# KerkDovan/univer-ocr

Measured on AMD Instinct MI355X. Metric: document-images/sec (fwd+bwd) on 256x512 synthetic pages, higher is better.
Workload: dtype f32; 1 GPU; BASELINE configs[2]: my_model train step (fwd+loss+bwd+L2+SGD) of Monochrome+Paragraph+Line on (32,256,512,1) pages and Char on (32,32,64,1) line strips per GPU; batch_per_gpu=32, global_batch=32, optimizer=sgd, parallelism=dp1, h2d_inclusive=False, input_grads=True, hip_graphs=True, pipelined_lanes=True, hw_queues=4

## Files before the change

include/univer_hip.h:

```cpp
#ifndef UNIVER_HIP_H
#define UNIVER_HIP_H

#include <stddef.h>
#include <stdint.h>

#ifdef __cplusplus
extern "C" {
#endif

#define UOCR_ABI_VERSION 4

typedef struct uocr_ctx uocr_ctx;

enum { UOCR_F32 = 0, UOCR_F64 = 1, UOCR_F16 = 2 };
#define UOCR_F16_SCALED(k) (UOCR_F16 | ((k) << 8))
#define UOCR_DTYPE_BASE(dtype) ((dtype) & 0xff)
#define UOCR_DTYPE_GRAD_SCALE_LOG2(dtype) (((dtype) >> 8) & 0xff)
enum { UOCR_ACT_NONE = 0, UOCR_ACT_RELU = 1, UOCR_ACT_LEAKY = 2, UOCR_ACT_SIGMOID = 3 };
enum { UOCR_LOSS_DICE = 0, UOCR_LOSS_JACCARD = 1 };
enum {
    UOCR_OK = 0,
    UOCR_ERR_ARG = -1,
    UOCR_ERR_DTYPE = -2,
    UOCR_ERR_HIP = -3,
    UOCR_ERR_WORKSPACE = -4,
    UOCR_ERR_UNSUPPORTED = -5,
    UOCR_ERR_RCCL = -6
};

int uocr_abi_version(void);
int uocr_ctx_create(int device, size_t workspace_bytes, uocr_ctx** out);
int uocr_ctx_create_cu_mask(int device, size_t workspace_bytes, const uint32_t* cu_mask, int mask_words, uocr_ctx** out);
int uocr_ctx_destroy(uocr_ctx* ctx);
int uocr_ctx_set_stream(uocr_ctx* ctx, void* hip_stream);
void* uocr_ctx_get_stream(uocr_ctx* ctx);
int uocr_ctx_set_option(uocr_ctx* ctx, const char* key, int value);
int uocr_ctx_last_split(uocr_ctx* ctx, int* blocks, long long* items);
int uocr_ctx_last_gemm(uocr_ctx* ctx, int* bm, int* gm, int* gn, int* nsplit);
int uocr_ctx_last_gemm_group(uocr_ctx* ctx, int* problems, int* split_problems);
int uocr_ctx_last_pair(uocr_ctx* ctx, int* kernel, int* g, int* mode, int* pf, int* nw, int* blocks_x, int* bands,
                       int* band_h);
enum {
    UOCR_CONV_NONE = 0,
    UOCR_CONV_GENERIC = 1,
    UOCR_CONV_MFMA = 2,
    UOCR_CONV_H16 = 3,
    UOCR_CONV_H16_WGRAD = 4,
    UOCR_CONV_H16_WGRAD_S2 = 5,
    UOCR_CONV_T32 = 6,
    UOCR_CONV_T32_WGRAD = 7,
    UOCR_CONV_H3 = 8,
    UOCR_CONV_TILED = 9,
    UOCR_CONV_C16_EXPAND = 10,
    UOCR_CONV_C16_REDUCE = 11,
    UOCR_CONV_C16_WGRAD = 12,
    UOCR_CONV_DGRAD_S2 = 13,
    UOCR_CONV_DGRAD_C64S2 = 14,
    UOCR_CONV_WGRAD_T542 = 15,
    UOCR_CONV_WGRAD_S2_TILED = 16,
    UOCR_CONV_TABLE_FAST = 17,
    UOCR_CONV_TABLE_PX = 18
};
int uocr_ctx_last_conv(uocr_ctx* ctx, int* entry, int* kernel);
int uocr_ctx_reserve_workspace(uocr_ctx* ctx, size_t bytes);
const char* uocr_last_error(uocr_ctx* ctx);
int uocr_malloc(uocr_ctx* ctx, size_t bytes, void** out);
int uocr_free(uocr_ctx* ctx, void* ptr);
int uocr_memset_zero(uocr_ctx* ctx, void* ptr, size_t bytes);
int uocr_h2d(uocr_ctx* ctx, void* dst, const void* src_host, size_t bytes);
int uocr_d2h_sync(uocr_ctx* ctx, void* dst_host, const void* src, size_t bytes);
int uocr_d2d(uocr_ctx* ctx, void* dst, const void* src, size_t bytes);
int uocr_stream_sync(uocr_ctx* ctx);
// ... 140 lines not shown
```

univer-ocr_amd/csrc/ctx.hip:

```cpp
#include <cstdlib>

#include "finish_group.h"
#include "gemm.h"
#include "uocr_common.h"

extern "C" {

int uocr_abi_version(void) { return UOCR_ABI_VERSION; }

int uocr_ctx_create(int device, size_t workspace_bytes, uocr_ctx** out) {
    if (!out || device < 0) return UOCR_ERR_ARG;
    *out = nullptr;
    int count = 0;
    if (hipGetDeviceCount(&count) != hipSuccess || device >= count) return UOCR_ERR_HIP;
    if (hipSetDevice(device) != hipSuccess) return UOCR_ERR_HIP;
    uocr_ctx* ctx = new uocr_ctx();
    ctx->device = device;
    ctx->err[0] = 0;
    ctx->workspace = nullptr;
    ctx->workspace_bytes = 0;
    ctx->sync = nullptr;
    ctx->gemm_defer = nullptr;
    ctx->snap_src = nullptr;
    ctx->snap_count = 0;
    ctx->snap_ring = nullptr;
    ctx->snap_ring_len = 0;
    ctx->snap_counter = nullptr;
    ctx->finish_defer = nullptr;
    ctx->owns_stream = true;
    ctx->opt_mfma = 1;
    ctx->opt_fast = 1;
    ctx->opt_tiled = 1;
    ctx->opt_split = 1024;
    ctx->opt_split_min = 3;
    ctx->opt_bm = 0;
    ctx->opt_h16 = 1;
    ctx->opt_t32 = 2;
    ctx->opt_xcd = 1;
    ctx->opt_pair_band = 0;
    ctx->opt_pair_g = 4;
    ctx->opt_group_blocks = 0;
    ctx->opt_wgrad_bands = 0;
    ctx->opt_max_blocks = 0;
    ctx->split_blocks = 0;
    ctx->split_items = 0;
    ctx->gemm_bm = ctx->gemm_gm = ctx->gemm_gn = ctx->gemm_nsplit = 0;
    ctx->gemm_group_count = ctx->gemm_group_split = 0;
    uocr_note_pair(ctx, 0, 0, 0, 0, 0, 0, 0, 0);
    uocr_note_conv(ctx, 0, UOCR_CONV_NONE);
    ctx->opt_h3 = 0;
#ifdef UOCR_EXPERIMENTS
    if (const char* e = getenv("UOCR_H3")) ctx->opt_h3 = atoi(e);
#endif
    ctx->opt_pair_pf = -1;
    if (const char* e = getenv("UOCR_PAIR_PF")) ctx->opt_pair_pf = atoi(e);
    if (const char* e = getenv("UOCR_WGRAD_BANDS")) ctx->opt_wgrad_bands = atoi(e);
    if (hipStreamCreateWithFlags(&ctx->stream, hipStreamNonBlocking) != hipSuccess) {
        delete ctx;
        return UOCR_ERR_HIP;
    }
    hipDeviceProp_t prop;
    ctx->cu_count = 256;
    if (hipGetDeviceProperties(&prop, device) == hipSuccess) ctx->cu_count = prop.multiProcessorCount;
    if (workspace_bytes) {
        if (hipMalloc(&ctx->workspace, workspace_bytes) != hipSuccess) {
            hipStreamDestroy(ctx->stream);
            delete ctx;
            return UOCR_ERR_HIP;
        }
        ctx->workspace_bytes = workspace_bytes;
    }
    if (hipMalloc((void**)&ctx->sync, UOCR_SYNC_WORDS * sizeof(unsigned)) != hipSuccess ||
        hipMemsetAsync(ctx->sync, 0, UOCR_SYNC_WORDS * sizeof(unsigned), ctx->stream) != hipSuccess ||
        hipStreamSynchronize(ctx->stream) != hipSuccess) {
        if (ctx->sync) hipFree(ctx->sync);
        if (ctx->workspace) hipFree(ctx->workspace);
        hipStreamDestroy(ctx->stream);
        delete ctx;
        return UOCR_ERR_HIP;
    }
// ... 22 lines not shown

int uocr_ctx_destroy(uocr_ctx* ctx) {
    UOCR_CHECK_CTX(ctx);
    hipSetDevice(ctx->device);
    hipStreamSynchronize(ctx->stream);
    if (ctx->workspace) hipFree(ctx->workspace);
    if (ctx->sync) hipFree(ctx->sync);
    uocr_gemm_defer_free(ctx);
    uocr_finish_defer_free(ctx);
    if (ctx->owns_stream) hipStreamDestroy(ctx->stream);
    delete ctx;
    return UOCR_OK;
}

int uocr_ctx_set_stream(uocr_ctx* ctx, void* hip_stream) {
    UOCR_CHECK_CTX(ctx);
    if (ctx->owns_stream) {
        UOCR_HIP(ctx, hipStreamSynchronize(ctx->stream));
        UOCR_HIP(ctx, hipStreamDestroy(ctx->stream));
        ctx->owns_stream = false;
    }
    ctx->stream = (hipStream_t)hip_stream;
    return UOCR_OK;
}

int uocr_ctx_set_option(uocr_ctx* ctx, const char* key, int value) {
    UOCR_CHECK_CTX(ctx);
    UOCR_REQUIRE(ctx, key != nullptr);
    if (!strcmp(key, "mfma")) ctx->opt_mfma = value;
    else if (!strcmp(key, "fast_paths")) ctx->opt_fast = value;
    else if (!strcmp(key, "tiled")) ctx->opt_tiled = value;
    else if (!strcmp(key, "split_blocks")) ctx->opt_split = value;
    else if (!strcmp(key, "split_min")) ctx->opt_split_min = value;
    else if (!strcmp(key, "gemm_bm")) ctx->opt_bm = value;
    else if (!strcmp(key, "xcd_remap")) ctx->opt_xcd = value;
    else if (!strcmp(key, "h16")) ctx->opt_h16 = value;
    else if (!strcmp(key, "t32")) {
        if (value & ~UOCR_T32_BUILT)
            UOCR_FAIL(ctx, UOCR_ERR_UNSUPPORTED, "option t32 = %d asks for kernels this library was built without "
                      "(UOCR_BUILD_EXPERIMENTS=1 ./build.sh)", value);
        ctx->opt_t32 = value;
    }
    else if (!strcmp(key, "pair_band")) ctx->opt_pair_band = value;
    else if (!strcmp(key, "pair_g")) ctx->opt_pair_g = value;
    else if (!strcmp(key, "group_blocks")) ctx->opt_group_blocks = value;
    else if (!strcmp(key, "wgrad_bands") && value >= 0) ctx->opt_wgrad_bands = value;
    else if (!strcmp(key, "max_blocks") && value >= 0) ctx->opt_max_blocks = value;
    else if (!strcmp(key, "h3")) {
#ifndef UOCR_EXPERIMENTS
        if (value) UOCR_FAIL(ctx, UOCR_ERR_UNSUPPORTED, "option h3: this library was built without conv_h3 "
                             "(UOCR_BUILD_EXPERIMENTS=1 ./build.sh)");
#endif
        ctx->opt_h3 = value;
    }
    else if (!strcmp(key, "pair_pf")) ctx->opt_pair_pf = value;
    else UOCR_FAIL(ctx, UOCR_ERR_ARG, "unknown option '%s'", key);
    return UOCR_OK;
}

int uocr_ctx_last_split(uocr_ctx* ctx, int* blocks, long long* items) {
    UOCR_CHECK_CTX(ctx);
    UOCR_REQUIRE(ctx, blocks && items);
    *blocks = ctx->split_blocks;
    *items = ctx->split_items;
    return UOCR_OK;
}

int uocr_ctx_last_gemm(uocr_ctx* ctx, int* bm, int* gm, int* gn, int* nsplit) {
    UOCR_CHECK_CTX(ctx);
    UOCR_REQUIRE(ctx, bm && gm && gn && nsplit);
    *bm = ctx->gemm_bm;
    *gm = ctx->gemm_gm;
    *gn = ctx->gemm_gn;
    *nsplit = ctx->gemm_nsplit;
    return UOCR_OK;
}

int uocr_ctx_last_gemm_group(uocr_ctx* ctx, int* problems, int* split_problems) {
    UOCR_CHECK_CTX(ctx);
    UOCR_REQUIRE(ctx, problems && split_problems);
    *problems = ctx->gemm_group_count;
    *split_problems = ctx->gemm_group_split;
    return UOCR_OK;
}

int uocr_ctx_last_pair(uocr_ctx* ctx, int* kernel, int* g, int* mode, int* pf, int* nw, int* blocks_x, int* bands,
                       int* band_h) {
    UOCR_CHECK_CTX(ctx);
    UOCR_REQUIRE(ctx, kernel && g && mode && pf && nw && blocks_x && bands && band_h);
    *kernel = ctx->pair_kernel;
    *g = ctx->pair_g;
    *mode = ctx->pair_mode;
    *pf = ctx->pair_pf;
    *nw = ctx->pair_nw;
    *blocks_x = ctx->pair_blocks_x;
    *bands = ctx->pair_bands;
    *band_h = ctx->pair_band_h;
    return UOCR_OK;
}

int uocr_ctx_last_conv(uocr_ctx* ctx, int* entry, int* kernel) {
    UOCR_CHECK_CTX(ctx);
    UOCR_REQUIRE(ctx, entry && kernel);
    *entry = ctx->conv_entry;
    *kernel = ctx->conv_kernel;
    return UOCR_OK;
}

void* uocr_ctx_get_stream(uocr_ctx* ctx) { return ctx ? (void*)ctx->stream : nullptr; }

int uocr_ctx_reserve_workspace(uocr_ctx* ctx, size_t bytes) {
    UOCR_CHECK_CTX(ctx);
    if (bytes <= ctx->workspace_bytes) return UOCR_OK;
    UOCR_HIP(ctx, hipSetDevice(ctx->device));
    UOCR_HIP(ctx, hipStreamSynchronize(ctx->stream));
    if (ctx->workspace) UOCR_HIP(ctx, hipFree(ctx->workspace));
    ctx->workspace = nullptr;
    ctx->workspace_bytes = 0;
// ... 146 lines not shown
```

univer-ocr_amd/csrc/gemm_mfma.hip:

```cpp
#include <array>
#include <type_traits>

#include "conv_dims.h"
#include "gemm.h"

namespace {

using f32x16 = __attribute__((ext_vector_type(16))) float;

constexpr int BN = 64;
constexpr int BD = 32;
constexpr int LDA = BD + 1;

struct alignas(16) F4 {
    float v[4];
};

__device__ __forceinline__ F4 f4_zero() { return F4{{0.f, 0.f, 0.f, 0.f}}; }
__device__ __forceinline__ F4 f4_fill(float x) { return F4{{x, x, x, x}}; }

enum : int { LD_KEEP = 0, LD_ZERO = 1, LD_E0 = 2, LD_PAD = 3 };

__device__ __forceinline__ F4 ld_resolve(F4 v, int code, float pad) {
    const float first = code == LD_PAD ? pad : (code == LD_E0 ? 1.f : 0.f);
    const float rest = code == LD_PAD ? pad : 0.f;
    F4 r;
    r.v[0] = code == LD_KEEP ? v.v[0] : first;
#pragma unroll
    for (int q = 1; q < 4; ++q) r.v[q] = code == LD_KEEP ? v.v[q] : rest;
    return r;
}

struct FastDiv {
    unsigned mul, shift;
    int d;
    FastDiv() = default;
    explicit FastDiv(int divisor) : mul(0), shift(0), d(divisor) {
        if (divisor > 1) {
            int lg = 0;
            while ((1ll << lg) < divisor) ++lg;
            const int p = 31 + lg;
// ... 306 lines not shown
            if (c.oy == d.oh) {
                c.oy = 0;
                c.b += 1;
                c.base += (d.h - d.oh * d.sh) * d.w * d.cin;
            }
        }
    }
    __device__ __forceinline__ F4 load_at(const Row& r, const Cursor& c, int& code) const {
        const int iy = c.oy * d.sh - d.ph + r.ky, ix = c.ox * d.sw - d.pw + r.kx;
        const bool inside = (unsigned)iy < (unsigned)d.h && (unsigned)ix < (unsigned)d.w;
        code = (c.b >= d.n || r.kind == 2) ? LD_ZERO : (r.kind == 1 ? LD_E0 : (inside ? LD_KEEP : LD_PAD));
        const int off = c.base + ((r.ky - d.ph) * d.w + (r.kx - d.pw)) * d.cin + r.ic0;
        return *reinterpret_cast<const F4*>(x + (code == LD_KEEP ? off : 0));
    }
};

template <int BM>
constexpr int gemm_a_floats() { return 2 * BM * LDA; }
template <typename BLoader>
constexpr int gemm_b_floats() { return 2 * (BLoader::DEPTH_CONTIG ? BN * LDA : BD * BN); }

__device__ __forceinline__ void gemm_block_coords(int lin, int gx, int gy, int gz, int xcd_remap, int& bx, int& by, int& bz) {
    if (xcd_remap) {
        const int total = gx * gy * gz;
        const int c = lin & 7, q = total >> 3, r = total & 7;
        lin = c * q + min(c, r) + (lin >> 3);
    }
    bx = lin % gx;
    const int rest = lin / gx;
    by = rest % gy;
    bz = rest / gy;
}

template <int BM, typename ALoader, typename BLoader>
__device__ __forceinline__ void gemm_tile(const ALoader& A, const BLoader& B, const Epilogue& ep, int M, int N, int ntiles,
                                          int tiles_per_split, float* slabs, int bx, int by, int bz, float* As,
                                          float* Bs) {
    constexpr int WM = BM / 32;
    constexpr int WN = 4 / WM;
    constexpr int NB = (BN / WN) / 32;
    constexpr int A_PASSES = BM / 32;
    constexpr int AM_GROUPS = BM / 4;
    constexpr int AM_ROWS = 256 / AM_GROUPS;
    constexpr int AM_PASSES = BD / AM_ROWS;
    constexpr int A_REGS = ALoader::DEPTH_CONTIG ? A_PASSES : AM_PASSES;
    constexpr int ASZ = BM * LDA;
    constexpr int BSZ = BLoader::DEPTH_CONTIG ? BN * LDA : BD * BN;

    const int tid = threadIdx.x, lane = tid & 63, wave = tid >> 6;
    const int m0 = bx * BM, n0 = by * BN;
    const int t_begin = bz * tiles_per_split;
    const int t_end = min(ntiles, t_begin + tiles_per_split);

    typename ALoader::Row rows[ALoader::DEPTH_CONTIG ? A_PASSES : 1];
    int a_kq = 0, a_r = 0, a_iq = 0, a_pr = 0;
    if constexpr (ALoader::DEPTH_CONTIG) {
        a_kq = tid & 7;
        a_r = tid >> 3;
#pragma unroll
        for (int s = 0; s < A_PASSES; ++s) rows[s] = A.prep(m0 + a_r + 32 * s);
    } else {
        a_iq = tid % AM_GROUPS;
        a_pr = tid / AM_GROUPS;
        rows[0] = A.prep(m0 + a_iq * 4);
    }
    const int b_nq = tid & 15, b_kr = tid >> 4;
    const int b_kq = tid & 7, b_r = tid >> 3;

    F4 areg[A_REGS], breg[2];
    int acode[A_REGS], bcode[2];
// ... 121 lines not shown
        if (band_live) {
            int ia = buf * ASZ + (ALoader::DEPTH_CONTIG ? fi * LDA + fk : fk * BM + fi);
            int ib = buf * BSZ + (BLoader::DEPTH_CONTIG ? fj * LDA + fk : fk * BN + fj);
            asm volatile("" : "+v"(ia), "+v"(ib));
            auto frag_a = [&](int k) { return As[ia + (ALoader::DEPTH_CONTIG ? k : k * BM)]; };
            auto frag_b = [&](int k, int nb) {
                return Bs[ib + (BLoader::DEPTH_CONTIG ? nb * 32 * LDA + k : k * BN + nb * 32)];
            };
            float a = frag_a(0), b[NB];
#pragma unroll
            for (int nb = 0; nb < NB; ++nb) b[nb] = frag_b(0, nb);
#pragma unroll
            for (int k = 0; k < BD; k += 2) {
                float an = 0.f, bn[NB];
                if (k + 2 < BD) {
                    an = frag_a(k + 2);
#pragma unroll
                    for (int nb = 0; nb < NB; ++nb) bn[nb] = frag_b(k + 2, nb);
                }
#pragma unroll
                for (int nb = 0; nb < NB; ++nb) acc[nb] = __builtin_amdgcn_mfma_f32_32x32x2f32(a, b[nb], acc[nb], 0, 0, 0);
                if (k + 2 < BD) {
                    a = an;
#pragma unroll
                    for (int nb = 0; nb < NB; ++nb) b[nb] = bn[nb];
                }
            }
        }
        if (more) store_tile(buf ^ 1);
        __syncthreads();
        t = tn;
    }

#pragma unroll
    for (int nb = 0; nb < NB; ++nb) {
        const int j = n0 + fj + nb * 32;
#pragma unroll
        for (int r = 0; r < 16; ++r) {
            const int i = m0 + wm * 32 + (r & 3) + 8 * (r >> 2) + 4 * (lane >> 5);
            if (i < M && j < N) {
                if (slabs) slabs[((long)bz * M + i) * N + j] = acc[nb][r];
                else epilogue_store(ep, i, j, acc[nb][r]);
            }
        }
    }
}

template <int BM, typename ALoader, typename BLoader>
__global__ __launch_bounds__(256) void mfma_gemm_kernel(ALoader A, BLoader B, Epilogue ep, int M, int N,
                                                        int ntiles, int tiles_per_split, float* slabs,
                                                        int xcd_remap) {
    __shared__ __attribute__((aligned(16))) float As[gemm_a_floats<BM>()];
    __shared__ __attribute__((aligned(16))) float Bs[gemm_b_floats<BLoader>()];
    int bx, by, bz;
    gemm_block_coords(blockIdx.x + gridDim.x * (blockIdx.y + gridDim.y * blockIdx.z), gridDim.x, gridDim.y, gridDim.z,
                      xcd_remap, bx, by, bz);
    gemm_tile<BM, ALoader, BLoader>(A, B, ep, M, N, ntiles, tiles_per_split, slabs, bx, by, bz, As, Bs);
}

__global__ __launch_bounds__(256) void slab_reduce_kernel(const float* __restrict__ slabs, int nsplit, int M, int N,
                                                          Epilogue ep) {
    const long total = (long)M * N;
    for (long idx = (long)blockIdx.x * blockDim.x + threadIdx.x; idx < total; idx += (long)gridDim.x * blockDim.x) {
        float v = 0.f;
        int z = 0;
        for (; z + 8 <= nsplit; z += 8) {
            float t[8];
#pragma unroll
            for (int k = 0; k < 8; ++k) t[k] = slabs[(long)(z + k) * total + idx];
#pragma unroll
            for (int k = 0; k < 8; ++k) v += t[k];
        }
        for (; z < nsplit; ++z) v += slabs[(long)z * total + idx];
        epilogue_store(ep, (int)(idx / N), (int)(idx % N), v);
    }
}

__global__ __launch_bounds__(256) void transpose_kernel(const float* __restrict__ in, float* __restrict__ out,
                                                        int rows, int cols) {
    const long total = (long)rows * cols;
    for (long idx = (long)blockIdx.x * blockDim.x + threadIdx.x; idx < total; idx += (long)gridDim.x * blockDim.x) {
        const int c = (int)(idx / rows), r = (int)(idx % rows);
        out[idx] = in[(long)r * cols + c];
    }
}

inline bool aligned16(const void* p) { return (reinterpret_cast<uintptr_t>(p) & 15u) == 0; }

inline float* ws_slabs(uocr_ctx* ctx) { return (float*)ctx->workspace; }
inline float* ws_aux(uocr_ctx* ctx) { return (float*)((char*)ctx->workspace + ctx->workspace_bytes / 2); }
inline size_t ws_half(uocr_ctx* ctx) { return ctx->workspace_bytes / 2; }

template <typename ALoader, typename BLoader>
int launch_mfma(uocr_ctx* ctx, const ALoader& A, const BLoader& B, const Epilogue& ep, int M, int N, int depth,
                bool allow_split) {
    const int ntiles = (depth + BD - 1) / BD;
    const long tiles128 = (long)((M + 127) / 128) * ((N + BN - 1) / BN);
    const long deep = (allow_split && ctx->opt_split > 0) ? min(256, ntiles / 32) : 1;
    int bm = (tiles128 >= 512 || tiles128 * deep >= 512) ? 128 : 64;
    if (ctx->opt_bm == 64 || ctx->opt_bm == 128) bm = ctx->opt_bm;
    const int gm = (M + bm - 1) / bm, gn = (N + BN - 1) / BN;
    int nsplit = 1;
    const int target = ctx->opt_split == 1024 ? ctx->cu_count * (bm == 128 ? 3 : 4) : ctx->opt_split;
    if (allow_split && target > 0 && gm * gn < target && ntiles >= 4) {
        nsplit = ctx->opt_split == 1024 ? max(1, target / (gm * gn)) : (target + gm * gn - 1) / (gm * gn);
        const int cap = max(min(32, ntiles / 2), min(256, ntiles / 32));
        if (nsplit > cap) nsplit = cap;
        const size_t per = (size_t)M * N * sizeof(float);
        if ((size_t)nsplit * per > ws_half(ctx)) nsplit = (int)(ws_half(ctx) / per);
        if (nsplit < 1) nsplit = 1;
        if (nsplit < ctx->opt_split_min) nsplit = 1;
    }
    const int tps = (ntiles + nsplit - 1) / nsplit;
    nsplit = (ntiles + tps - 1) / tps;
    float* slabs = nsplit > 1 ? ws_slabs(ctx) : nullptr;
    ctx->gemm_bm = bm;
    ctx->gemm_gm = gm;
    ctx->gemm_gn = gn;
    ctx->gemm_nsplit = nsplit;
    const dim3 grid(gm, gn, nsplit), block(256);
    if (bm == 128)
        hipLaunchKernelGGL((mfma_gemm_kernel<128, ALoader, BLoader>), grid, block, 0, ctx->stream, A, B, ep, M, N, ntiles, tps,
                           slabs, ctx->opt_xcd);
    else
        hipLaunchKernelGGL((mfma_gemm_kernel<64, ALoader, BLoader>), grid, block, 0, ctx->stream, A, B, ep, M, N, ntiles, tps,
                           slabs, ctx->opt_xcd);
    UOCR_LAUNCH_CHECK(ctx);
    if (nsplit > 1) {
        hipLaunchKernelGGL(slab_reduce_kernel, dim3(uocr_blocks_for((size_t)M * N, 256, 1024)), dim3(256), 0,
                           ctx->stream, (const float*)slabs, nsplit, M, N, ep);
        UOCR_LAUNCH_CHECK(ctx);
    }
    return UOCR_OK;
}

constexpr int GROUP_MAX = 8, GROUP_MAX_TYPE = 4;

struct GroupShape {
    int M, N, ntiles, tps, gx, gy, gz, first_block;
    float* slabs;
    Epilogue ep;
};
struct GroupArgs {
    int count, xcd_remap;
    int type[GROUP_MAX];
    int index[GROUP_MAX];
    GroupShape shape[GROUP_MAX];
    BRowMajor b[GROUP_MAX];
    AConvWgrad conv_a[GROUP_MAX_TYPE];
    AColMajor col_a[GROUP_MAX_TYPE];
};

__global__ __launch_bounds__(256) void mfma_gemm_group_kernel(GroupArgs g) {
    __shared__ __attribute__((aligned(16))) float As[gemm_a_floats<64>()];
    __shared__ __attribute__((aligned(16))) float Bs[gemm_b_floats<BRowMajor>()];
    int p = 0;
    while (p + 1 < g.count && (int)blockIdx.x >= g.shape[p + 1].first_block) ++p;
    const GroupShape& sh = g.shape[p];
    int bx, by, bz;
    gemm_block_coords((int)blockIdx.x - sh.first_block, sh.gx, sh.gy, sh.gz, g.xcd_remap, bx, by, bz);
    if (g.type[p] == 0)
        gemm_tile<64, AConvWgrad, BRowMajor>(g.conv_a[g.index[p]], g.b[p], sh.ep, sh.M, sh.N, sh.ntiles, sh.tps, sh.slabs, bx,
                                             by, bz, As, Bs);
    else
        gemm_tile<64, AColMajor, BRowMajor>(g.col_a[g.index[p]], g.b[p], sh.ep, sh.M, sh.N, sh.ntiles, sh.tps, sh.slabs, bx,
                                            by, bz, As, Bs);
}

struct GroupReduceArgs {
    int count;
    long first[GROUP_MAX + 1];
    const float* slabs[GROUP_MAX];
    int nsplit[GROUP_MAX], N[GROUP_MAX];
    Epilogue ep[GROUP_MAX];
};

__global__ __launch_bounds__(256) void slab_reduce_group_kernel(GroupReduceArgs a) {
    const long total = a.first[a.count];
    for (long g = (long)blockIdx.x * blockDim.x + threadIdx.x; g < total; g += (long)gridDim.x * blockDim.x) {
        int p = 0;
        while (p + 1 < a.count && g >= a.first[p + 1]) ++p;
        const long idx = g - a.first[p], size = a.first[p + 1] - a.first[p];
        const float* slabs = a.slabs[p];
        const int nsplit = a.nsplit[p];
        float v = 0.f;
        int z = 0;
        for (; z + 8 <= nsplit; z += 8) {
            float t[8];
#pragma unroll
            for (int k = 0; k < 8; ++k) t[k] = slabs[(long)(z + k) * size + idx];
#pragma unroll
            for (int k = 0; k < 8; ++k) v += t[k];
        }
        for (; z < nsplit; ++z) v += slabs[(long)z * size + idx];
        epilogue_store(a.ep[p], (int)(idx / a.N[p]), (int)(idx % a.N[p]), v);
    }
}

struct GemmDefer {
// ... 61 lines not shown
    GemmDefer* d = defer_of(ctx);
    if (!d || d->count == 0) return UOCR_OK;
    GroupArgs& g = d->args;
    g.count = d->count;
    g.xcd_remap = ctx->opt_xcd;
    double work[GROUP_MAX], total_work = 0.0;
    for (int p = 0; p < g.count; ++p) {
        GroupShape& sh = g.shape[p];
        sh.gx = (sh.M + 63) / 64;
        sh.gy = (sh.N + BN - 1) / BN;
        sh.ntiles = (d->depth[p] + BD - 1) / BD;
        work[p] = (double)sh.gx * sh.gy * sh.ntiles;
        total_work += work[p];
    }
    const double target = ctx->opt_split <= 0 ? 0.0 : ctx->opt_group_blocks > 0 ? (double)ctx->opt_group_blocks : 4.0 * ctx->cu_count;
    size_t slab_floats = 0;
    int nblocks = 0;
    GroupReduceArgs r{};
    for (int p = 0; p < g.count; ++p) {
        GroupShape& sh = g.shape[p];
        const int tiles = sh.gx * sh.gy;
        int nsplit = (int)(target * work[p] / total_work / tiles + 0.5);
        const int cap = std::max(std::min(32, sh.ntiles / 2), std::min(256, sh.ntiles / 32));
        nsplit = std::max(1, std::min(nsplit, cap));
        const size_t per = (size_t)sh.M * sh.N;
        while (nsplit > 1 && (slab_floats + (size_t)nsplit * per) * sizeof(float) > ws_half(ctx)) --nsplit;
        if (nsplit < ctx->opt_split_min) nsplit = 1;
        sh.tps = (sh.ntiles + nsplit - 1) / nsplit;
        nsplit = (sh.ntiles + sh.tps - 1) / sh.tps;
        sh.gz = nsplit;
        sh.first_block = nblocks;
        nblocks += tiles * nsplit;
        sh.slabs = nullptr;
        if (nsplit > 1) {
            sh.slabs = ws_slabs(ctx) + slab_floats;
            slab_floats += (size_t)nsplit * per;
            const int q = r.count++;
            r.first[q + 1] = r.first[q] + (long)per;
            r.slabs[q] = sh.slabs;
            r.nsplit[q] = nsplit;
            r.N[q] = sh.N;
            r.ep[q] = sh.ep;
        }
    }
    int max_split = 1;
    for (int p = 0; p < g.count; ++p) max_split = std::max(max_split, g.shape[p].gz);
    ctx->gemm_bm = 64;
    ctx->gemm_gm = ctx->gemm_gn = 0;
    ctx->gemm_nsplit = max_split;
    ctx->gemm_group_count = g.count;
    ctx->gemm_group_split = r.count;
    hipLaunchKernelGGL(mfma_gemm_group_kernel, dim3(nblocks), dim3(256), 0, ctx->stream, g);
    UOCR_LAUNCH_CHECK(ctx);
    if (r.count > 0) {
        hipLaunchKernelGGL(slab_reduce_group_kernel, dim3(uocr_blocks_for((size_t)r.first[r.count], 256, 2048)), dim3(256),
                           0, ctx->stream, r);
        UOCR_LAUNCH_CHECK(ctx);
    }
    d->count = d->nconv = d->ncol = 0;
    return UOCR_OK;
}

inline Epilogue plain_epilogue(float* c, long ldc, int accumulate) {
    return Epilogue{c, ldc, nullptr, UOCR_ACT_NONE, 0.f, accumulate, -1, nullptr, nullptr, UOCR_ACT_NONE, 0.f};
}

}

bool uocr_gemm_mfma_eligible(uocr_ctx* ctx, int dtype, const GemmArgs& g) {
    if (dtype != UOCR_F32 || ctx->opt_mfma == 0) return false;
    const bool a_row = (g.a_cs == 1), a_col = (g.a_rs == 1 && !a_row);
    if (!(a_row || a_col)) return false;
    if (!(g.b_cs == 1 || g.b_rs == 1)) return false;
    if (g.b_cs != 1 && (g.b_cs != g.depth || (size_t)g.n * g.depth * sizeof(float) > ws_half(ctx))) return false;
    if (ctx->opt_mfma == 2) return true;
    return (double)g.m * g.n * g.depth >= 4.0e6 && g.n >= 32 && g.m >= 32;
}

int uocr_gemm_mfma(uocr_ctx* ctx, const GemmArgs& g) {
    Epilogue ep0 = plain_epilogue((float*)g.c, g.ldc, g.accumulate);
    ep0.act = g.act;
    ep0.alpha = (float)g.act_alpha;
    ep0.mask_y = (const float*)g.mask_y;
    ep0.mask_act = g.mask_act;
// ... 111 lines not shown
```

univer-ocr_amd/csrc/uocr_common.h:

```cpp
#pragma once
#include <hip/hip_runtime.h>
#include <stdint.h>
#include <stdio.h>
#include <string.h>

#include "univer_hip.h"

struct uocr_ctx {
    int device;
    hipStream_t stream;
    bool owns_stream;
    void* workspace;
    size_t workspace_bytes;
    const double* snap_src;
    int snap_count;
    double* snap_ring;
    int snap_ring_len;
    unsigned* snap_counter;
    void* gemm_defer;
    void* finish_defer;
    unsigned* sync;
    int cu_count;
    int opt_mfma;
    int opt_fast;
    int opt_tiled;
    int opt_split;
    int opt_split_min;
    int opt_xcd;
    int opt_bm;
    int opt_h16;
    int opt_t32;
    int opt_pair_band;
    int opt_pair_pf;
    int opt_h3;
    int opt_group_blocks;
    int opt_wgrad_bands;
    int opt_pair_g;
    int opt_max_blocks;
    int split_blocks;
    long long split_items;
    int gemm_bm, gemm_gm, gemm_gn, gemm_nsplit;
    int gemm_group_count, gemm_group_split;
    int pair_kernel, pair_g, pair_mode, pair_pf;
    int pair_nw, pair_blocks_x, pair_bands, pair_band_h;
    int conv_entry, conv_kernel;
    int label_th, label_tw, label_launches;
    char err[512];
};

constexpr int UOCR_SYNC_WORDS = 1 << 18;
#ifdef UOCR_EXPERIMENTS
constexpr int UOCR_T32_BUILT = 255;
#else
constexpr int UOCR_T32_BUILT = 2;
#endif

#define UOCR_FAIL(ctx, code, ...)                                   \
    do {                                                            \
        if (ctx) snprintf((ctx)->err, sizeof((ctx)->err), __VA_ARGS__); \
        return (code);                                              \
    } while (0)

#define UOCR_HIP(ctx, call)                                                              \
    do {                                                                                 \
        hipError_t e_ = (call);                                                          \
        if (e_ != hipSuccess)                                                            \
            UOCR_FAIL(ctx, UOCR_ERR_HIP, "%s failed: %s (%s:%d)", #call, hipGetErrorString(e_), \
                      __FILE__, __LINE__);                                               \
    } while (0)

#define UOCR_LAUNCH_CHECK(ctx)                                                           \
    do {                                                                                 \
        hipError_t e_ = hipGetLastError();                                               \
        if (e_ != hipSuccess)                                                            \
            UOCR_FAIL(ctx, UOCR_ERR_HIP, "kernel launch failed: %s (%s:%d)", hipGetErrorString(e_), \
// ... 254 lines not shown
```

univer-ocr_amd/hip/lib.py:

```python
import ctypes as C
import os

_HERE = os.path.dirname(os.path.abspath(__file__))
_LIB_NAME = 'libuniver_hip.so'

F32, F64, F16 = 0, 1, 2
DP_UNIQUE_ID_BYTES = 128


def f16_scaled(k):
    return F16 | (int(k) << 8)
ACT_NONE, ACT_RELU, ACT_LEAKY, ACT_SIGMOID = 0, 1, 2, 3
LOSS_DICE, LOSS_JACCARD = 0, 1
THRESH_MEAN, THRESH_MEAN_MAX, THRESH_VALUE = 0, 1, 2
CONV_KERNELS = ('none', 'generic', 'mfma', 'h16', 'h16_wgrad', 'h16_wgrad_s2', 't32', 't32_wgrad', 'h3', 'tiled',
                'c16_expand', 'c16_reduce', 'c16_wgrad', 'dgrad_s2', 'dgrad_c64s2', 'wgrad_t542', 'wgrad_s2_tiled',
                'table_fast', 'table_px')


class HipError(RuntimeError):
    pass


def lib_path():
    return os.path.join(os.path.dirname(_HERE), _LIB_NAME)


def dtype_code(np_dtype):
    import numpy as np
    dt = np.dtype(np_dtype)
    if dt == np.float32:
        return F32
    if dt == np.float64:
        return F64
    if dt == np.float16:
        return F16
    raise HipError(f'unsupported dtype {dt}: the HIP backend stores float16 / float32 / float64')


_vp, _i, _d, _sz = C.c_void_p, C.c_int, C.c_double, C.c_size_t
_ctx = C.c_void_p

_PROTOS = {
    'uocr_ctx_create': [_i, _sz, C.POINTER(_ctx)],
    'uocr_ctx_create_cu_mask': [_i, _sz, C.POINTER(C.c_uint32), _i, C.POINTER(_ctx)],
    'uocr_ctx_destroy': [_ctx],
    'uocr_ctx_set_stream': [_ctx, _vp],
    'uocr_ctx_reserve_workspace': [_ctx, _sz],
    'uocr_ctx_set_option': [_ctx, C.c_char_p, _i],
    'uocr_ctx_last_split': [_ctx, C.POINTER(_i), C.POINTER(C.c_longlong)],
    'uocr_ctx_last_gemm': [_ctx, C.POINTER(_i), C.POINTER(_i), C.POINTER(_i), C.POINTER(_i)],
    'uocr_ctx_last_gemm_group': [_ctx, C.POINTER(_i), C.POINTER(_i)],
    'uocr_ctx_last_pair': [_ctx] + [C.POINTER(_i)] * 8,
    'uocr_ctx_last_conv': [_ctx, C.POINTER(_i), C.POINTER(_i)],
    'uocr_malloc': [_ctx, _sz, C.POINTER(_vp)],
    'uocr_free': [_ctx, _vp],
    'uocr_memset_zero': [_ctx, _vp, _sz],
    'uocr_h2d': [_ctx, _vp, _vp, _sz],
    'uocr_d2h_sync': [_ctx, _vp, _vp, _sz],
    'uocr_d2d': [_ctx, _vp, _vp, _sz],
    'uocr_stream_sync': [_ctx],
    'uocr_event_create': [C.POINTER(_vp)],
    'uocr_event_destroy': [_vp],
    'uocr_event_record': [_ctx, _vp],
    'uocr_stream_wait_event': [_ctx, _vp],
    'uocr_event_elapsed_ms_sync': [_vp, _vp, C.POINTER(C.c_float)],
    'uocr_event_synchronize': [_vp],
    'uocr_graph_begin_capture': [_ctx],
    'uocr_graph_end_capture': [_ctx, C.POINTER(_vp)],
    'uocr_graph_launch': [_ctx, _vp],
    'uocr_graph_destroy': [_vp],
    'uocr_ctx_set_loss_snapshot': [_ctx, _vp, _i, _vp, _i, _vp],
    'uocr_wgrad_defer_begin': [_ctx],
    'uocr_wgrad_defer_flush': [_ctx, _i],
    'uocr_device_info': [_ctx, C.c_char_p, _sz, C.POINTER(_i), C.POINTER(_sz)],
    'uocr_conv2d_fwd': [_ctx, _i, _vp, _vp, _vp, _vp] + [_i] * 13 + [_d, _i, _i, _d],
    'uocr_conv2d_bwd_data': [_ctx, _i, _vp, _vp, _vp] + [_i] * 13 + [_vp, _i, _d],
    'uocr_conv2d_bwd_weight': [_ctx, _i, _vp, _vp, _vp, _vp] + [_i] * 13 + [_d, _i, _i],
    'uocr_conv_pair_fwd': [_ctx, _i] + [_vp] * 6 + [_i] * 4 + [_d, _i, _i, _d, _i],
    'uocr_conv_pair_bwd': [_ctx, _i] + [_vp] * 11 + [_i] * 4 + [_d, _i, _i, _d, _i, _i],
    'uocr_upconv2x_fwd': [_ctx, _i, _vp, _vp, _vp, _vp] + [_i] * 9 + [_i, _i, _d, _vp],
    'uocr_upconv2x_bwd_data': [_ctx, _i, _vp, _vp, _vp] + [_i] * 9 + [_vp, _i, _d, _vp],
    'uocr_upconv2x_bwd_weight': [_ctx, _i, _vp, _vp, _vp, _vp] + [_i] * 9 + [_i, _i],
    'uocr_maxpool2d_fwd': [_ctx, _i, _vp, _vp, _vp] + [_i] * 12,
    'uocr_maxpool2d_bwd': [_ctx, _i, _vp, _vp, _vp] + [_i] * 12,
# ... 78 lines not shown
```

univer-ocr_amd/nn/gpu.py:

```python
import os

import numpy as np
os.environ.setdefault('GPU_MAX_HW_QUEUES', '8')

import torch

from ..hip import lib as hiplib
from ..hip.lib import HipError

_TORCH_DT = {np.dtype(np.float32): torch.float32, np.dtype(np.float64): torch.float64,
             np.dtype(np.float16): torch.float16,
             np.dtype(np.uint8): torch.uint8, np.dtype(np.int32): torch.int32, np.dtype(np.int64): torch.int64}
_CODE = {torch.float32: hiplib.F32, torch.float64: hiplib.F64, torch.float16: hiplib.F16}
_NP_DT = {v: k for k, v in _TORCH_DT.items()}


class Runtime:

    def __init__(self, device_index=None):
        if not torch.cuda.is_available():
            raise HipError('no HIP device visible: the univer-ocr MI355X backend has no host fallback')
        self.lib = hiplib.get_lib()
        if device_index is None:
            device_index = int(os.environ.get('LOCAL_RANK', '0')) % max(1, torch.cuda.device_count())
# ... 63 lines not shown
    def use_stream(self, torch_stream):
        import ctypes as C
        self.call('uocr_ctx_set_stream', C.c_void_p(torch_stream.cuda_stream))

    def set_option(self, key, value):
        current = self.ctx
        try:
            for handle in [h for h, _ in self._lanes] + [s.handle for s in self._sides.values()]:
                self.ctx = handle
                self.call('uocr_ctx_set_option', key.encode(), int(value))
        finally:
            self.ctx = current
        self._options = getattr(self, '_options', {})
        self._options[key] = int(value)

    def last_split(self):
        import ctypes as C
        blocks, items = C.c_int(), C.c_longlong()
        self.call('uocr_ctx_last_split', C.byref(blocks), C.byref(items))
        return blocks.value, items.value

    def last_gemm(self):
        import ctypes as C
        v = [C.c_int() for _ in range(4)]
        self.call('uocr_ctx_last_gemm', *[C.byref(x) for x in v])
        return tuple(x.value for x in v)

    def last_gemm_group(self):
        import ctypes as C
        problems, split = C.c_int(), C.c_int()
        self.call('uocr_ctx_last_gemm_group', C.byref(problems), C.byref(split))
        return problems.value, split.value

    def last_pair(self):
        import ctypes as C
        v = [C.c_int() for _ in range(8)]
        self.call('uocr_ctx_last_pair', *[C.byref(x) for x in v])
        return tuple(x.value for x in v)

    def last_conv(self):
        import ctypes as C
        entry, kernel = C.c_int(), C.c_int()
        self.call('uocr_ctx_last_conv', C.byref(entry), C.byref(kernel))
        return entry.value, kernel.value

    def last_label(self):
        import ctypes as C
        v = [C.c_int() for _ in range(3)]
        self.call('uocr_ctx_last_label', *[C.byref(x) for x in v])
        return tuple(x.value for x in v)

    def set_loss_snapshot(self, arena):
        if arena is None:
            self.call('uocr_ctx_set_loss_snapshot', None, 0, None, 0, None)
        else:
            self.call('uocr_ctx_set_loss_snapshot', arena.array.ptr, arena.array.shape[0], arena.ring.ptr, arena.ring_len,
                      arena.counter.ptr)

    def defer_wgrad(self):
        return _DeferScope(self)

    def keep(self, *arrays):
        held = self._deferred.get(self.ctx.value)
        if held is not None:
            held.extend(arrays)

# ... 510 lines not shown
```

Baseline: 32220 images/s.

## Fuse split-K slab reduction into MFMA GEMM via per-tile atomic tickets

Split-K GEMMs, both single and grouped, now write per-tile partial slabs with sc1 buffer stores and take an atomic ticket per output tile. The last-arriving block sums all slabs and runs the epilogue, so no separate slab_reduce kernel is launched when nsplit is at most 8. This removes a kernel launch and a full reread of the slabs per split GEMM. In exchange it adds atomics, a fence and a serialized reduction tail in one block per tile, and it relies on counters being cleared in workspace sync memory.

```diff
diff --git a/include/univer_hip.h b/include/univer_hip.h
--- a/include/univer_hip.h
+++ b/include/univer_hip.h
@@ -38,6 +38,7 @@
 int uocr_ctx_last_split(uocr_ctx* ctx, int* blocks, long long* items);
 int uocr_ctx_last_gemm(uocr_ctx* ctx, int* bm, int* gm, int* gn, int* nsplit);
 int uocr_ctx_last_gemm_group(uocr_ctx* ctx, int* problems, int* split_problems);
+int uocr_ctx_last_gemm_fused(uocr_ctx* ctx, int* fused);
 int uocr_ctx_last_pair(uocr_ctx* ctx, int* kernel, int* g, int* mode, int* pf, int* nw, int* blocks_x, int* bands,
                        int* band_h);
 enum {
diff --git a/univer-ocr_amd/csrc/ctx.hip b/univer-ocr_amd/csrc/ctx.hip
--- a/univer-ocr_amd/csrc/ctx.hip
+++ b/univer-ocr_amd/csrc/ctx.hip
@@ -33,6 +33,7 @@
     ctx->opt_tiled = 1;
     ctx->opt_split = 1024;
     ctx->opt_split_min = 3;
+    ctx->opt_split_fused = 8;
     ctx->opt_bm = 0;
     ctx->opt_h16 = 1;
     ctx->opt_t32 = 2;
@@ -46,6 +47,7 @@
     ctx->split_items = 0;
     ctx->gemm_bm = ctx->gemm_gm = ctx->gemm_gn = ctx->gemm_nsplit = 0;
     ctx->gemm_group_count = ctx->gemm_group_split = 0;
+    ctx->gemm_fused = 0;
     uocr_note_pair(ctx, 0, 0, 0, 0, 0, 0, 0, 0);
     uocr_note_conv(ctx, 0, UOCR_CONV_NONE);
     ctx->opt_h3 = 0;
@@ -134,6 +136,7 @@
     else if (!strcmp(key, "tiled")) ctx->opt_tiled = value;
     else if (!strcmp(key, "split_blocks")) ctx->opt_split = value;
     else if (!strcmp(key, "split_min")) ctx->opt_split_min = value;
+    else if (!strcmp(key, "split_fused") && value >= 0) ctx->opt_split_fused = value;
     else if (!strcmp(key, "gemm_bm")) ctx->opt_bm = value;
     else if (!strcmp(key, "xcd_remap")) ctx->opt_xcd = value;
     else if (!strcmp(key, "h16")) ctx->opt_h16 = value;
@@ -186,6 +189,13 @@
     return UOCR_OK;
 }
 
+int uocr_ctx_last_gemm_fused(uocr_ctx* ctx, int* fused) {
+    UOCR_CHECK_CTX(ctx);
+    UOCR_REQUIRE(ctx, fused);
+    *fused = ctx->gemm_fused;
+    return UOCR_OK;
+}
+
 int uocr_ctx_last_pair(uocr_ctx* ctx, int* kernel, int* g, int* mode, int* pf, int* nw, int* blocks_x, int* bands,
                        int* band_h) {
     UOCR_CHECK_CTX(ctx);
diff --git a/univer-ocr_amd/csrc/gemm_mfma.hip b/univer-ocr_amd/csrc/gemm_mfma.hip
--- a/univer-ocr_amd/csrc/gemm_mfma.hip
+++ b/univer-ocr_amd/csrc/gemm_mfma.hip
@@ -7,6 +7,8 @@
 namespace {
 
 using f32x16 = __attribute__((ext_vector_type(16))) float;
+using f32x4 = __attribute__((ext_vector_type(4))) float;
+using u32x4 = __attribute__((ext_vector_type(4))) uint32_t;
 
 constexpr int BN = 64;
 constexpr int BD = 32;
@@ -379,10 +381,23 @@
     bz = rest / gy;
 }
 
+struct SplitFuse {
+    unsigned* counters;
+    int nsplit;
+    int gm, tiles;
+};
+
+__device__ __forceinline__ void slab_store_sc1(__amdgpu_buffer_rsrc_t r, int byte_off, f32x4 v) {
+    __builtin_amdgcn_raw_buffer_store_b128(__builtin_bit_cast(u32x4, v), r, byte_off, 0, 16);
+}
+__device__ __forceinline__ f32x4 slab_load_sc1(__amdgpu_buffer_rsrc_t r, int byte_off) {
+    return __builtin_bit_cast(f32x4, __builtin_amdgcn_raw_buffer_load_b128(r, byte_off, 0, 16));
+}
+
 template <int BM, typename ALoader, typename BLoader>
 __device__ __forceinline__ void gemm_tile(const ALoader& A, const BLoader& B, const Epilogue& ep, int M, int N, int ntiles,
-                                          int tiles_per_split, float* slabs, int bx, int by, int bz, float* As,
-                                          float* Bs) {
+                                          int tiles_per_split, float* slabs, const SplitFuse& fuse, int bx, int by, int bz,
+                                          float* As, float* Bs) {
     constexpr int WM = BM / 32;
     constexpr int WN = 4 / WM;
     constexpr int NB = (BN / WN) / 32;
@@ -570,6 +585,72 @@
         t = tn;
     }
 
+    if (fuse.counters) {
+        constexpr int TILE_BYTES = BM * BN * (int)sizeof(float);
+        const int tile = by * fuse.gm + bx;
+        const int slot = ((wn * WM + wm) * 64 + lane) * 16;
+        auto slab_of = [&](int z) {
+            return __builtin_amdgcn_make_buffer_rsrc(slabs + ((long)z * fuse.tiles + tile) * (BM * BN), 0, TILE_BYTES, 0x00020000);
+        };
+        if (band_live) {
+            const auto mine = slab_of(bz);
+#pragma unroll
+            for (int nb = 0; nb < NB; ++nb)
+#pragma unroll
+                for (int g = 0; g < 4; ++g) {
+                    const f32x4 v = {acc[nb][4 * g], acc[nb][4 * g + 1], acc[nb][4 * g + 2], acc[nb][4 * g + 3]};
+                    slab_store_sc1(mine, (nb * 4 + g) * 4096 + slot, v);
+                }
+        }
+        asm volatile("s_waitcnt vmcnt(0)" ::: "memory");
+        __syncthreads();
+        if (tid == 0) {
+            const unsigned ticket = __hip_atomic_fetch_add(fuse.counters + tile, 1u, __ATOMIC_RELAXED, __HIP_MEMORY_SCOPE_AGENT);
+            As[0] = ticket == (unsigned)fuse.nsplit - 1u ? 1.f : 0.f;
+        }
+        __syncthreads();
+        if (As[0] == 0.f) return;
+        __builtin_amdgcn_fence(__ATOMIC_ACQUIRE, "wavefront");
+        if (band_live) {
+#pragma unroll
+            for (int nb = 0; nb < NB; ++nb) {
+                f32x4 sum[4];
+#pragma unroll
+                for (int g = 0; g < 4; ++g) sum[g] = f32x4{0.f, 0.f, 0.f, 0.f};
+                auto add_slabs = [&](int z, auto count) {
+                    constexpr int K = decltype(count)::value;
+                    f32x4 t[K][4];
+#pragma unroll
+                    for (int k = 0; k < K; ++k) {
+                        const auto r = slab_of(z + k);
+#pragma unroll
+                        for (int g = 0; g < 4; ++g) t[k][g] = slab_load_sc1(r, (nb * 4 + g) * 4096 + slot);
+                    }
+#pragma unroll
+                    for (int k = 0; k < K; ++k)
+#pragma unroll
+                        for (int g = 0; g < 4; ++g) sum[g] += t[k][g];
+                };
+                int z = 0;
+                for (; z + 4 <= fuse.nsplit; z += 4) add_slabs(z, std::integral_constant<int, 4>{});
+                if (z + 2 <= fuse.nsplit) {
+                    add_slabs(z, std::integral_constant<int, 2>{});
+                    z += 2;
+                }
+                if (z < fuse.nsplit) add_slabs(z, std::integral_constant<int, 1>{});
+                const int j = n0 + fj + nb * 32;
+#pragma unroll
+                for (int g = 0; g < 4; ++g)
+#pragma unroll
+                    for (int q = 0; q < 4; ++q) {
+                        const int i = m0 + wm * 32 + q + 8 * g + 4 * (lane >> 5);
+                        if (i < M && j < N) epilogue_store(ep, i, j, sum[g][q]);
+                    }
+            }
+        }
+        if (tid == 0) sync_clear(fuse.counters + tile);
+        return;
+    }
 #pragma unroll
     for (int nb = 0; nb < NB; ++nb) {
         const int j = n0 + fj + nb * 32;
@@ -587,13 +668,13 @@
 template <int BM, typename ALoader, typename BLoader>
 __global__ __launch_bounds__(256) void mfma_gemm_kernel(ALoader A, BLoader B, Epilogue ep, int M, int N,
                                                         int ntiles, int tiles_per_split, float* slabs,
-                                                        int xcd_remap) {
+                                                        SplitFuse fuse, int xcd_remap) {
     __shared__ __attribute__((aligned(16))) float As[gemm_a_floats<BM>()];
     __shared__ __attribute__((aligned(16))) float Bs[gemm_b_floats<BLoader>()];
     int bx, by, bz;
     gemm_block_coords(blockIdx.x + gridDim.x * (blockIdx.y + gridDim.y * blockIdx.z), gridDim.x, gridDim.y, gridDim.z,
                       xcd_remap, bx, by, bz);
-    gemm_tile<BM, ALoader, BLoader>(A, B, ep, M, N, ntiles, tiles_per_split, slabs, bx, by, bz, As, Bs);
+    gemm_tile<BM, ALoader, BLoader>(A, B, ep, M, N, ntiles, tiles_per_split, slabs, fuse, bx, by, bz, As, Bs);
 }
 
 __global__ __launch_bounds__(256) void slab_reduce_kernel(const float* __restrict__ slabs, int nsplit, int M, int N,
@@ -628,6 +709,12 @@
 inline float* ws_slabs(uocr_ctx* ctx) { return (float*)ctx->workspace; }
 inline float* ws_aux(uocr_ctx* ctx) { return (float*)((char*)ctx->workspace + ctx->workspace_bytes / 2); }
 inline size_t ws_half(uocr_ctx* ctx) { return ctx->workspace_bytes / 2; }
+
+constexpr int GEMM_SYNC_BASE = 1024, GEMM_SYNC_WORDS = 4096;
+constexpr int GROUP_SYNC_BASE = 8192, GROUP_SYNC_WORDS = 4096;
+static_assert(GROUP_SYNC_BASE >= GEMM_SYNC_BASE + GEMM_SYNC_WORDS && GROUP_SYNC_BASE + GROUP_SYNC_WORDS <= UOCR_SYNC_WORDS);
+
+inline bool fuse_allowed(uocr_ctx* ctx, int nsplit) { return nsplit > 1 && nsplit <= ctx->opt_split_fused; }
 
 template <typename ALoader, typename BLoader>
 int launch_mfma(uocr_ctx* ctx, const ALoader& A, const BLoader& B, const Epilogue& ep, int M, int N, int depth,
@@ -652,19 +739,23 @@
     const int tps = (ntiles + nsplit - 1) / nsplit;
     nsplit = (ntiles + tps - 1) / tps;
     float* slabs = nsplit > 1 ? ws_slabs(ctx) : nullptr;
+    const bool fused = fuse_allowed(ctx, nsplit) && gm * gn <= GEMM_SYNC_WORDS &&
+                       (size_t)nsplit * gm * gn * bm * BN * sizeof(float) <= ws_half(ctx);
+    const SplitFuse fuse{fused ? ctx->sync + GEMM_SYNC_BASE : nullptr, nsplit, gm, gm * gn};
     ctx->gemm_bm = bm;
     ctx->gemm_gm = gm;
     ctx->gemm_gn = gn;
     ctx->gemm_nsplit = nsplit;
+    ctx->gemm_fused = fused ? 1 : 0;
     const dim3 grid(gm, gn, nsplit), block(256);
     if (bm == 128)
         hipLaunchKernelGGL((mfma_gemm_kernel<128, ALoader, BLoader>), grid, block, 0, ctx->stream, A, B, ep, M, N, ntiles, tps,
-                           slabs, ctx->opt_xcd);
+                           slabs, fuse, ctx->opt_xcd);
     else
         hipLaunchKernelGGL((mfma_gemm_kernel<64, ALoader, BLoader>), grid, block, 0, ctx->stream, A, B, ep, M, N, ntiles, tps,
-                           slabs, ctx->opt_xcd);
+                           slabs, fuse, ctx->opt_xcd);
     UOCR_LAUNCH_CHECK(ctx);
-    if (nsplit > 1) {
+    if (nsplit > 1 && !fused) {
         hipLaunchKernelGGL(slab_reduce_kernel, dim3(uocr_blocks_for((size_t)M * N, 256, 1024)), dim3(256), 0,
                            ctx->stream, (const float*)slabs, nsplit, M, N, ep);
         UOCR_LAUNCH_CHECK(ctx);
@@ -677,6 +768,7 @@
 struct GroupShape {
     int M, N, ntiles, tps, gx, gy, gz, first_block;
     float* slabs;
+    unsigned* counters;
     Epilogue ep;
 };
 struct GroupArgs {
@@ -697,12 +789,13 @@
     const GroupShape& sh = g.shape[p];
     int bx, by, bz;
     gemm_block_coords((int)blockIdx.x - sh.first_block, sh.gx, sh.gy, sh.gz, g.xcd_remap, bx, by, bz);
+    const SplitFuse fuse{sh.counters, sh.gz, sh.gx, sh.gx * sh.gy};
     if (g.type[p] == 0)
-        gemm_tile<64, AConvWgrad, BRowMajor>(g.conv_a[g.index[p]], g.b[p], sh.ep, sh.M, sh.N, sh.ntiles, sh.tps, sh.slabs, bx,
-                                             by, bz, As, Bs);
+        gemm_tile<64, AConvWgrad, BRowMajor>(g.conv_a[g.index[p]], g.b[p], sh.ep, sh.M, sh.N, sh.ntiles, sh.tps, sh.slabs,
+                                             fuse, bx, by, bz, As, Bs);
     else
-        gemm_tile<64, AColMajor, BRowMajor>(g.col_a[g.index[p]], g.b[p], sh.ep, sh.M, sh.N, sh.ntiles, sh.tps, sh.slabs, bx,
-                                            by, bz, As, Bs);
+        gemm_tile<64, AColMajor, BRowMajor>(g.col_a[g.index[p]], g.b[p], sh.ep, sh.M, sh.N, sh.ntiles, sh.tps, sh.slabs,
+                                            fuse, bx, by, bz, As, Bs);
 }
 
 struct GroupReduceArgs {
@@ -830,16 +923,36 @@
         sh.first_block = nblocks;
         nblocks += tiles * nsplit;
         sh.slabs = nullptr;
-        if (nsplit > 1) {
-            sh.slabs = ws_slabs(ctx) + slab_floats;
-            slab_floats += (size_t)nsplit * per;
-            const int q = r.count++;
-            r.first[q + 1] = r.first[q] + (long)per;
-            r.slabs[q] = sh.slabs;
-            r.nsplit[q] = nsplit;
-            r.N[q] = sh.N;
-            r.ep[q] = sh.ep;
-        }
+        sh.counters = nullptr;
+        if (nsplit > 1) slab_floats += (size_t)nsplit * per;
+    }
+    size_t rest = slab_floats, used = 0;
+    int counters = 0, fused_count = 0, split_count = 0;
+    for (int p = 0; p < g.count; ++p) {
+        GroupShape& sh = g.shape[p];
+        if (sh.gz <= 1) continue;
+        ++split_count;
+        const int tiles = sh.gx * sh.gy;
+        const size_t per = (size_t)sh.M * sh.N, plain = (size_t)sh.gz * per, padded = (size_t)sh.gz * tiles * 64 * BN;
+        rest -= plain;
+        const size_t start = (used + 3) & ~(size_t)3;
+        if (fuse_allowed(ctx, sh.gz) && counters + tiles <= GROUP_SYNC_WORDS &&
+            (start + padded + rest) * sizeof(float) <= ws_half(ctx)) {
+            sh.slabs = ws_slabs(ctx) + start;
+            sh.counters = ctx->sync + GROUP_SYNC_BASE + counters;
+            counters += tiles;
+            used = start + padded;
+            ++fused_count;
+            continue;
+        }
+        sh.slabs = ws_slabs(ctx) + used;
+        used += plain;
+        const int q = r.count++;
+        r.first[q + 1] = r.first[q] + (long)per;
+        r.slabs[q] = sh.slabs;
+        r.nsplit[q] = sh.gz;
+        r.N[q] = sh.N;
+        r.ep[q] = sh.ep;
     }
     int max_split = 1;
     for (int p = 0; p < g.count; ++p) max_split = std::max(max_split, g.shape[p].gz);
@@ -847,7 +960,8 @@
     ctx->gemm_gm = ctx->gemm_gn = 0;
     ctx->gemm_nsplit = max_split;
     ctx->gemm_group_count = g.count;
-    ctx->gemm_group_split = r.count;
+    ctx->gemm_group_split = split_count;
+    ctx->gemm_fused = fused_count;
     hipLaunchKernelGGL(mfma_gemm_group_kernel, dim3(nblocks), dim3(256), 0, ctx->stream, g);
     UOCR_LAUNCH_CHECK(ctx);
     if (r.count > 0) {
diff --git a/univer-ocr_amd/csrc/uocr_common.h b/univer-ocr_amd/csrc/uocr_common.h
--- a/univer-ocr_amd/csrc/uocr_common.h
+++ b/univer-ocr_amd/csrc/uocr_common.h
@@ -26,6 +26,7 @@
     int opt_tiled;
     int opt_split;
     int opt_split_min;
+    int opt_split_fused;
     int opt_xcd;
     int opt_bm;
     int opt_h16;
@@ -41,6 +42,7 @@
     long long split_items;
     int gemm_bm, gemm_gm, gemm_gn, gemm_nsplit;
     int gemm_group_count, gemm_group_split;
+    int gemm_fused;
     int pair_kernel, pair_g, pair_mode, pair_pf;
     int pair_nw, pair_blocks_x, pair_bands, pair_band_h;
     int conv_entry, conv_kernel;
diff --git a/univer-ocr_amd/hip/lib.py b/univer-ocr_amd/hip/lib.py
--- a/univer-ocr_amd/hip/lib.py
+++ b/univer-ocr_amd/hip/lib.py
@@ -51,6 +51,7 @@
     'uocr_ctx_last_split': [_ctx, C.POINTER(_i), C.POINTER(C.c_longlong)],
     'uocr_ctx_last_gemm': [_ctx, C.POINTER(_i), C.POINTER(_i), C.POINTER(_i), C.POINTER(_i)],
     'uocr_ctx_last_gemm_group': [_ctx, C.POINTER(_i), C.POINTER(_i)],
+    'uocr_ctx_last_gemm_fused': [_ctx, C.POINTER(_i)],
     'uocr_ctx_last_pair': [_ctx] + [C.POINTER(_i)] * 8,
     'uocr_ctx_last_conv': [_ctx, C.POINTER(_i), C.POINTER(_i)],
     'uocr_malloc': [_ctx, _sz, C.POINTER(_vp)],
diff --git a/univer-ocr_amd/nn/gpu.py b/univer-ocr_amd/nn/gpu.py
--- a/univer-ocr_amd/nn/gpu.py
+++ b/univer-ocr_amd/nn/gpu.py
@@ -119,6 +119,12 @@
         self.call('uocr_ctx_last_gemm_group', C.byref(problems), C.byref(split))
         return problems.value, split.value
 
+    def last_gemm_fused(self):
+        import ctypes as C
+        fused = C.c_int()
+        self.call('uocr_ctx_last_gemm_fused', C.byref(fused))
+        return fused.value
+
     def last_pair(self):
         import ctypes as C
         v = [C.c_int() for _ in range(8)]
```

After: 31360 images/s. 0.973x the previous value.
